# ziyu0425/PDE-Solver

Measured on NVIDIA B200. Metric: GDOF/s, higher is better.
Workload: dtype f64

## Files before the change

### pde_solver_b200/csrc/heat2.cu

```cuda
#include <cuda.h>

#include <cmath>

#include "device.cuh"
#include "tma.cuh"

namespace {

#ifndef H_RR_STAGES
#define H_RR_STAGES 3
#endif
template <bool RR>
struct HS { static constexpr int N = RR ? H_RR_STAGES : 4; };

template <int CW, int YSB>
struct HG {
  static constexpr int TX = CW - 2, YSA = YSB + 1, TY = 2 * YSB, RA = TY + 2;
  static constexpr int BX = TX + 4, BYX = TY + 4, BYB = TY + 2;
  static constexpr int XBOX = BX * BYX, BBOX = BX * BYB;
  static constexpr int XS = (XBOX + 15) / 16 * 16, BS = (BBOX + 15) / 16 * 16;
  static constexpr int STAGE = XS + BS;
  static constexpr int RING = RA * CW;
  static constexpr int NT = 2 * CW;
  static constexpr size_t smem(int nst) { return ((size_t)nst * STAGE + 4 * RING) * sizeof(double) + nst * sizeof(uint64_t); }
};

struct H2Coef {
  double c0, cxp, cxm, cyp, cym, czp, czm, cxyp, cxym, cxzp, cxzm, cyzp, cyzm, cdp, cdm;
};
struct H2Args {
  double* y;
  double a0, a1, k1;
  int do_reduce;
  double* yc;
  int cnn0, cnn1, cnzl, cz0, cPX;
  long long cplane;
};
struct H2Geom {
  int nn0, nn1, nzl, z0, nzg, PX;
  long long plane;
  int ntx, nty, nzc, zc;
};

template <int YS>
__device__ __forceinline__ void h2_contrib(const H2Coef& C, const double (&V)[YS + 2][3], double (&aP)[YS], double (&a0)[YS],
                                           double (&aM)[YS]) {
#pragma unroll
  for (int j = 0; j < YS; ++j) {
    const int r = j + 1;
    double t = fma(C.c0, V[r][1], a0[j]);
    t = fma(C.cxp, V[r][2], t);
    t = fma(C.cxm, V[r][0], t);
    t = fma(C.cyp, V[r + 1][1], t);
    t = fma(C.cym, V[r - 1][1], t);
    t = fma(C.cxyp, V[r + 1][2], t);
    a0[j] = fma(C.cxym, V[r - 1][0], t);
    double p = fma(C.czp, V[r][1], aP[j]);
    p = fma(C.cxzp, V[r][2], p);
    p = fma(C.cyzp, V[r + 1][1], p);
    aP[j] = fma(C.cdp, V[r + 1][2], p);
    double m = C.czm * V[r][1];
    m = fma(C.cxzm, V[r][0], m);
    m = fma(C.cyzm, V[r - 1][1], m);
    aM[j] = fma(C.cdm, V[r - 1][0], m);
  }
}

template <int CW, int YSB, bool RR>
__global__ void __launch_bounds__(2 * CW, CW == 64 ? ((RR && H_RR_STAGES == 3) ? 4 : (YSB >= 4 ? 3 : (YSB == 3 ? 4 : 5))) : 6)
k_heat_post2(const __grid_constant__ CUtensorMap tmx, const __grid_constant__ CUtensorMap tmb,
             const __grid_constant__ H2Coef C, const __grid_constant__ H2Args a, const __grid_constant__ H2Geom ge,
             ReduceBuf red, double* red_out) {
  using G = HG<CW, YSB>;
  constexpr int YSA = G::YSA;
  constexpr int H_STAGES = HS<RR>::N;
  extern __shared__ __align__(128) unsigned char smem_raw[];
  double* const stage0 = reinterpret_cast<double*>(smem_raw);
  double* const ring0 = stage0 + H_STAGES * G::STAGE;
  uint64_t* const bars = reinterpret_cast<uint64_t*>(ring0 + 4 * G::RING);

  const int t = threadIdx.x;
  const int item = blockIdx.x;
  const int itx = item % ge.ntx;
  const int ity = (item / ge.ntx) % ge.nty;
  const int izc = item / (ge.ntx * ge.nty);
  const int x0 = itx * G::TX, y0 = ity * G::TY;
  const int za = izc * ge.zc;
  const int zb = min(za + ge.zc, ge.nzl);
  const int nplanes = zb - za + 4;
  const uint32_t bar0 = smem_u32(bars);
  const uint32_t stg0 = smem_u32(stage0);
  constexpr uint32_t STAGE_BYTES = G::STAGE * 8;

  auto issue = [&](int n) {
    const uint32_t bar = bar0 + 8 * (n % H_STAGES);
    const uint32_t dst = stg0 + (n % H_STAGES) * STAGE_BYTES;
    mbar_expect_tx(bar, (uint32_t)((G::XBOX + (n >= 2 ? G::BBOX : 0)) * 8));
    tma_load_4d(dst, &tmx, x0 - 2, y0 - 2, za - 2 + n + PDE_NG, 0, bar);
    if (n >= 2) tma_load_4d(dst + G::XS * 8, &tmb, x0 - 2, y0 - 1, za - 3 + n + PDE_NG, 0, bar);
  };
  if (t == 0) {
#pragma unroll
    for (int s = 0; s < H_STAGES; ++s) mbar_init(bar0 + 8 * s, 1);
    asm volatile("fence.mbarrier_init.release.cluster;" ::: "memory");
  }
  __syncthreads();
  if (t == 0)
    for (int n = 0; n < 2 && n < nplanes; ++n) issue(n);

  const int c = t % CW;
  const int s = t / CW;
  const int ix = x0 - 1 + c;
  const int cB = min(max(c, 1), CW - 2);
  const bool xfree = ix >= 1 && ix <= ge.nn0 - 2;
  unsigned mAb = 0, mBb = 0, okB = 0;
#pragma unroll
  for (int j = 0; j < YSA; ++j) {
    const int iy = y0 - 1 + s * YSA + j;
    if (xfree && iy >= 1 && iy <= ge.nn1 - 2) mAb |= 1u << j;
  }
#pragma unroll
  for (int j = 0; j < YSB; ++j) {
    const int iy = y0 + s * YSB + j;
    const bool in = c >= 1 && c <= G::TX && ix < ge.nn0 && iy < ge.nn1;
    if (in) okB |= 1u << j;
    if (in && xfree && iy >= 1 && iy <= ge.nn1 - 2) mBb |= 1u << j;
  }
  const int offA = (s * YSA) * G::BX + c;
  const int offbA = G::XS + (s * YSA) * G::BX + c + 1;
  const int offbB = G::XS + (s * YSB + 1) * G::BX + cB + 1;
  const int offxB = (s * YSB + 2) * G::BX + cB + 1;
  const int ringA = (s * YSA) * CW + c;
  const int ringB = (s * YSB) * CW + cB - 1;
  double* yrun = a.y + ((long long)ge.PX * (y0 + s * YSB) + ix) + ge.plane * za;

  double aA[YSA], aB[YSA], aC[YSA];
  double bA_[YSB], bB_[YSB], bC_[YSB];
#pragma unroll
  for (int j = 0; j < YSA; ++j) aA[j] = aB[j] = aC[j] = 0.0;
#pragma unroll
  for (int j = 0; j < YSB; ++j) bA_[j] = bB_[j] = bC_[j] = 0.0;
  double red_by = 0.0;

  auto body = [&](int i, double (&aP)[YSA], double (&a0)[YSA], double (&aM)[YSA], double (&bP)[YSB], double (&b0)[YSB],
                  double (&bM)[YSB]) {
    const int stage = i % H_STAGES;
    const int q = za - 2 + i;
    const int pA = q - 1;
    const int pB = q - 2;
    const bool finA = i >= 2, finB = i >= 4;
    double xB0[YSB], bvB[YSB];
    if (!RR && finB) {
      const double* const sx2 = stage0 + ((i - 2) % H_STAGES) * G::STAGE + offxB;
      const double* const sb1 = stage0 + ((i - 1) % H_STAGES) * G::STAGE + offbB;
#pragma unroll
      for (int j = 0; j < YSB; ++j) { xB0[j] = sx2[j * G::BX]; bvB[j] = sb1[j * G::BX]; }
    }
    mbar_wait(bar0 + 8 * stage, (uint32_t)((i / H_STAGES) & 1));
    const double* const sx = stage0 + stage * G::STAGE;
    {
      double V[YSA + 2][3];
      const double* const sp = sx + offA;
#pragma unroll
      for (int r = 0; r < YSA + 2; ++r)
#pragma unroll
        for (int cc = 0; cc < 3; ++cc)
          V[r][cc] = ((r == 0 && cc == 2) || (r == YSA + 1 && cc == 0)) ? 0.0 : sp[r * G::BX + cc];
      h2_contrib<YSA>(C, V, aP, a0, aM);
    }
    if (finA) {
      const int gz = pA + ge.z0;
      const bool zfree = gz >= 1 && gz <= ge.nzg - 2;
      const unsigned mA = zfree ? mAb : 0u;
      double* const ds = ring0 + ((pA + 4) & 3) * G::RING + ringA;
      const double* const sb = sx + offbA;
#pragma unroll
      for (int j = 0; j < YSA; ++j) ds[j * CW] = ((mA >> j) & 1u) ? a.a0 * (sb[j * G::BX] - aP[j]) : 0.0;
    }
    __syncthreads();
    if (t == 0 && i + 2 < nplanes) issue(i + 2);
    if (!RR && finA) {
      double V[YSB + 2][3];
      const double* const rp = ring0 + ((pA + 4) & 3) * G::RING + ringB;
#pragma unroll
      for (int r = 0; r < YSB + 2; ++r)
#pragma unroll
        for (int cc = 0; cc < 3; ++cc)
          V[r][cc] = ((r == 0 && cc == 2) || (r == YSB + 1 && cc == 0)) ? 0.0 : rp[r * CW + cc];
      h2_contrib<YSB>(C, V, bP, b0, bM);
    }
    if (RR && finB) {
      const int gz = pB + ge.z0;
      const int Z = (gz >> 1) - a.cz0;
      constexpr int NCX = G::TX / 2, NCY = G::TY / 2;
      if (!(gz & 1) && Z >= 0 && Z < a.cnzl && t < NCX * NCY) {
        const int cx = t % NCX, cy = t / NCX;
        const int X = (x0 >> 1) + cx, Y = (y0 >> 1) + cy;
        if (X < a.cnn0 && Y < a.cnn1) {
          const int o = (1 + 2 * cy) * CW + 1 + 2 * cx;
          const double* const r0 = ring0 + ((pB + 4) & 3) * G::RING + o;
          const double* const rm = ring0 + ((pB + 3) & 3) * G::RING + o;
          const double* const rp = ring0 + ((pB + 5) & 3) * G::RING + o;
          const double nb = ((r0[1] + r0[-1]) + (r0[CW] + r0[-CW])) + ((r0[CW + 1] + r0[-CW - 1]) + (rp[0] + rm[0])) +
                            ((rp[1] + rm[-1]) + (rp[CW] + rm[-CW])) + (rp[CW + 1] + rm[-CW - 1]);
          const int cgz = gz >> 1;
          const bool cfree = X >= 1 && X <= a.cnn0 - 2 && Y >= 1 && Y <= a.cnn1 - 2 && cgz >= 1 && cgz <= (ge.nzg >> 1) - 1;
          a.yc[(long long)a.cPX * Y + a.cplane * Z + X] = cfree ? fma(0.5, nb, r0[0]) : 0.0;
        }
      }
    }
    if (!RR && finB) {
      const int gz = pB + ge.z0;
      const bool zfree = gz >= 1 && gz <= ge.nzg - 2;
      const unsigned mB = zfree ? mBb : 0u;
      const double* const dso = ring0 + ((pB + 4) & 3) * G::RING + ringB + CW + 1;
#pragma unroll
      for (int j = 0; j < YSB; ++j) {
        const bool m = (mB >> j) & 1u;
        const double x2 = m ? fma(a.k1, dso[j * CW], fma(-a.a1, bP[j], xB0[j])) : xB0[j];
        if ((okB >> j) & 1u) yrun[j * (long long)ge.PX] = x2;
        red_by = fma(m ? bvB[j] : 0.0, x2, red_by);
      }
      yrun += ge.plane;
    }
  };

  for (int i = 0; i < nplanes; i += 3) {
    body(i, aA, aB, aC, bB_, bC_, bA_);
    if (i + 1 < nplanes) body(i + 1, aB, aC, aA, bC_, bA_, bB_);
    if (i + 2 < nplanes) body(i + 2, aC, aA, aB, bA_, bB_, bC_);
  }
  if (a.do_reduce) {
    double v[1] = {red_by};
    block_reduce_finalize<1>(v, red, red_out);
  }
}

template <int CW, int YSB, bool RR>
int launch_t(pde_ctx* c, const Grid& g, const OpDev& op, const double* x0, const double* b, const H2Args& ha_in) {
  using G = HG<CW, YSB>;
  H2Geom ge;
  ge.nn0 = g.nn[0]; ge.nn1 = g.nn[1]; ge.nzl = g.nzl; ge.z0 = g.z0; ge.nzg = g.nzg; ge.PX = g.PX; ge.plane = g.plane;
  ge.ntx = (g.nn[0] + G::TX - 1) / G::TX;
  ge.nty = (g.nn[1] + G::TY - 1) / G::TY;
  static const int zc_env = env_int("PDE_B200_P2_ZC", 64);
  int zc = zc_env < 4 ? 4 : zc_env;
  while (zc > 8 && (long long)ge.ntx * ge.nty * ((g.nzl + zc - 1) / zc) < 6LL * c->sm_count) zc /= 2;
  ge.nzc = (g.nzl + zc - 1) / zc;
  ge.zc = (g.nzl + ge.nzc - 1) / ge.nzc;
  ge.nzc = (g.nzl + ge.zc - 1) / ge.zc;
  const long long items = (long long)ge.ntx * ge.nty * ge.nzc;
  if (items > RED_MAX_BLOCKS) return 2;
  auto kern = k_heat_post2<CW, YSB, RR>;
  static bool attr_set = false;
  if (!attr_set) {
    CUDA_OK(cudaFuncSetAttribute(kern, cudaFuncAttributeMaxDynamicSharedMemorySize, (int)G::smem(HS<RR>::N)));
    CUDA_OK(cudaFuncSetAttribute(kern, cudaFuncAttributePreferredSharedMemoryCarveout, 100));
    attr_set = true;
  }
  CUtensorMap tmx, tmb;
  PDE_OK(field_tensor_map(x0, g, 1, G::BX, G::BYX, &tmx));
  PDE_OK(field_tensor_map(b, g, 1, G::BX, G::BYB, &tmb));
  H2Coef C;
  const double* h = op.h_int;
  C.c0 = h[0]; C.cxp = h[1]; C.cxm = h[2]; C.cyp = h[3]; C.cym = h[4]; C.czp = h[5]; C.czm = h[6]; C.cxyp = h[7];
  C.cxym = h[8]; C.cxzp = h[9]; C.cxzm = h[10]; C.cyzp = h[11]; C.cyzm = h[12]; C.cdp = h[13]; C.cdm = h[14];
  kern<<<(unsigned)items, G::NT, G::smem(HS<RR>::N), c->stream>>>(tmx, tmb, C, ha_in, ge, c->red, ha_in.do_reduce ? c->scal + ha_in.do_reduce - 1 : nullptr);
  c->launches++;
  CUDA_OK(cudaGetLastError());
  return 0;
}

bool heat2_applicable(const Grid& g, const OpDev& op) {
  static const int off = env_int("PDE_B200_NO_HEAT2", 0);
  if (off) return false;
  if (g.dim != 3 || g.nk != PDE_NOFF || op.ncomp != 1 || !op.uniform_diag) return false;
  return g.nn[0] >= 32 && g.nn[1] >= 8 && g.nzl >= 8;
}

template <bool RR>
int dispatch(pde_ctx* c, const Grid& g, const OpDev& op, const double* x0, const double* b, const H2Args& ha) {
  static const int cw_env = env_int("PDE_B200_P2_CW", 0);
  static const int ysb = env_int("PDE_B200_P2_YSB", 4);
  const int cw = cw_env ? cw_env : (g.nn[0] >= 128 ? 64 : 32);
  if (cw == 64 && ysb == 3) return launch_t<64, 3, RR>(c, g, op, x0, b, ha);
  if (cw == 64) return launch_t<64, 4, RR>(c, g, op, x0, b, ha);
  return launch_t<32, 4, RR>(c, g, op, x0, b, ha);
}

}

bool post2_applicable(const Grid& g, const OpDev& op) {
  if (g.dim != 3 || g.nk != PDE_NOFF || op.ncomp != 1 || !op.uniform_diag) return false;
  if (g.nn[0] < 32 || g.nn[1] < 8 || g.nzl < 8) return false;
  return !env_int("PDE_B200_NO_HEAT2", 0) || !env_int("PDE_B200_NO_POST2", 0);
}

int launch_heat_post2(pde_ctx* c, const Grid& g, const OpDev& op, const double* x0, const double* b, double* y, double c2_0,
                      double c1_1, double c2_1, int dot_slot, bool* handled) {
  *handled = false;
  if (!heat2_applicable(g, op) || !(c2_0 * op.h_dinv_int[0] > 0.0)) return 0;
  H2Args ha{};
  ha.y = y;
  ha.a0 = c2_0 * op.h_dinv_int[0];
  ha.a1 = c2_1 * op.h_dinv_int[0];
  ha.k1 = 1.0 + c1_1 + ha.a1 / ha.a0;
  ha.do_reduce = dot_slot >= 0 ? dot_slot + 1 : 0;
  const int rc = dispatch<false>(c, g, op, x0, b, ha);
  if (rc == 0) *handled = true;
  return rc == 2 ? 0 : rc;
}

int launch_heat_resid_restrict(pde_ctx* c, const Grid& gf, const Grid& gc, const OpDev& op, const double* x, const double* b,
                               double* bcoarse, bool* handled) {
  *handled = false;
  static const int off = env_int("PDE_B200_NO_RR", 0);
  if (off || !heat2_applicable(gf, op)) return 0;
  if (gf.nc[0] != 2 * gc.nc[0] || gf.nc[1] != 2 * gc.nc[1] || gf.nc[2] != 2 * gc.nc[2] || gf.z0 != 2 * gc.z0) return 0;
  H2Args ha{};
  ha.a0 = 1.0;
  ha.yc = bcoarse;
  ha.cnn0 = gc.nn[0]; ha.cnn1 = gc.nn[1]; ha.cnzl = gc.nzl; ha.cz0 = gc.z0; ha.cPX = gc.PX; ha.cplane = gc.plane;
  const int rc = dispatch<true>(c, gf, op, x, b, ha);
  if (rc == 0) *handled = true;
  return rc == 2 ? 0 : rc;
}
```

### pde_solver_b200/csrc/solver.cu

```cuda
#include <cmath>
#include <cstdio>
#include <cstdlib>
#include <cstring>

#include "solver.cuh"

int launch_stencil_generic(pde_ctx* c, const Grid& g, const BcDev& bc, const OpDev& op, const StencilArgs& a);
int launch_stencil_fast(pde_ctx* c, const Grid& g, const BcDev& bc, const OpDev& op, const StencilArgs& a, bool* handled);
int launch_heat_post2(pde_ctx* c, const Grid& g, const OpDev& op, const double* x0, const double* b, double* y, double c2_0,
                      double c1_1, double c2_1, int dot_slot, bool* handled);
bool elast3d_first2_ok(const Grid& g, const BcDev& bc, const OpDev& op);
bool post2_applicable(const Grid& g, const OpDev& op);
int launch_heat_resid_restrict(pde_ctx* c, const Grid& gf, const Grid& gc, const OpDev& op, const double* x, const double* b,
                               double* bcoarse, bool* handled);

int launch_stencil(pde_ctx* c, const Grid& g, const BcDev& bc, const OpDev& op, const StencilArgs& a) {
  if (a.variant == 0) {
    bool handled = false;
    PDE_OK(launch_stencil_fast(c, g, bc, op, a, &handled));
    if (handled) return 0;
  }
  return launch_stencil_generic(c, g, bc, op, a);
}

int Field::alloc(pde_ctx* c, const Grid& g, int ncomp) {
  release();
  const size_t lead = (((size_t)g.PX + 1 + 31) / 32) * 32;
  bytes = ((size_t)g.comp_stride * ncomp + 2 * lead) * sizeof(double);
  CUDA_OK(cudaMalloc(&raw, bytes));
  CUDA_OK(cudaMemsetAsync(raw, 0, bytes, c->stream));
  p = raw + lead + PDE_NG * g.plane;
  return 0;
}
void Field::release() {
  if (raw) cudaFree(raw);
  raw = p = nullptr;
  bytes = 0;
}

int Operator::upload(pde_ctx* c) {
  const int nc = tab.ncomp, nn = nc * nc;
  dev.ncomp = nc;
  dev.gershgorin = tab.gershgorin;
  std::vector<double> dinv((size_t)PDE_NCLASS * nc, 0.0);
  for (int cls = 0; cls < PDE_NCLASS; ++cls)
    for (int i = 0; i < nc; ++i) {
      double dg = tab.coef[((size_t)cls * PDE_NOFF + 0) * nn + i * nc + i];
      dinv[cls * nc + i] = dg > 0 ? 1.0 / dg : 0.0;
    }
  for (int k = 0; k < PDE_NOFF; ++k)
    for (int q = 0; q < nn; ++q) dev.h_int[k * nn + q] = tab.coef[((size_t)13 * PDE_NOFF + k) * nn + q];
  for (int i = 0; i < nc; ++i) dev.h_dinv_int[i] = dinv[13 * nc + i];
  dev.h_load_int = tab.load[13];
  {
    bool u = !bc.side_excl;
    for (int ax = 0; ax < 3; ++ax)
      if (g.nc[ax] > 0 && !(bc.on[2 * ax] && bc.on[2 * ax + 1])) u = false;
    dev.uniform_diag = u ? 1 : 0;
  }
  CUDA_OK(cudaMalloc(&dev.coef, tab.coef.size() * sizeof(double)));
  CUDA_OK(cudaMalloc(&dev.dinv, dinv.size() * sizeof(double)));
  CUDA_OK(cudaMalloc(&dev.load, PDE_NCLASS * sizeof(double)));
  CUDA_OK(cudaMemcpyAsync(dev.coef, tab.coef.data(), tab.coef.size() * sizeof(double), cudaMemcpyHostToDevice, c->stream));
  CUDA_OK(cudaMemcpyAsync(dev.dinv, dinv.data(), dinv.size() * sizeof(double), cudaMemcpyHostToDevice, c->stream));
  CUDA_OK(cudaMemcpyAsync(dev.load, tab.load.data(), PDE_NCLASS * sizeof(double), cudaMemcpyHostToDevice, c->stream));
  CUDA_OK(cudaStreamSynchronize(c->stream));
  return 0;
}
int Operator::setup_scalar(pde_ctx* c, const Grid& g_, const BcDev& bc_, double alpha, double beta) {
  release();
  g = g_;
  bc = bc_;
  PDE_OK(build_scalar_table(g.dim, g.h, g.nc, alpha, beta, &tab));
  return upload(c);
}
int Operator::setup_elasticity(pde_ctx* c, const Grid& g_, const BcDev& bc_, double lam, double mu) {
  release();
  g = g_;
  bc = bc_;
  PDE_OK(build_elasticity_table(g.dim, g.h, g.nc, lam, mu, &tab));
  return upload(c);
}
void Operator::release() {
  if (dev.coef) cudaFree(dev.coef);
  if (dev.dinv) cudaFree(dev.dinv);
  if (dev.load) cudaFree(dev.load);
  dev.coef = dev.dinv = dev.load = nullptr;
}

__global__ void k_publish_scal(const double* __restrict__ src, double* __restrict__ dst_host, int count) {
  if ((int)threadIdx.x < count) dst_host[threadIdx.x] = src[threadIdx.x];
  __threadfence_system();
}
// ... 172 lines not shown
  return 0;
}

int Hierarchy::build(pde_ctx* c, const Operator& fine, int kind, double p0, double p1) {
  release();
  const int dim = fine.g.dim;
  int ax[3], nax;
  internal_axes(dim, ax, &nax);
  int32_t n[3] = {0, 0, 0};
  double Lu[3] = {1, 1, 1};
  for (int q = 0; q < nax; ++q) {
    n[q] = fine.g.nc[ax[q]];
    Lu[q] = fine.g.h[ax[q]] * fine.g.nc[ax[q]];
  }
  const int ncomp = fine.tab.ncomp;
  static const long long rep_nodes = getenv("PDE_B200_REP_NODES") ? atoll(getenv("PDE_B200_REP_NODES")) : 400000;
  bool replicate = false;
  for (int level = 0;; ++level) {
    std::unique_ptr<MGLevel> L(new MGLevel());
    Grid g;
    if (c->world > 1 && level > 0 && !replicate) {
      long long gn = 1;
      for (int q = 0; q < nax; ++q) gn *= (n[q] + 1);
      replicate = gn <= rep_nodes;
    }
    if (replicate) {
      PDE_OK(make_grid(dim, n, Lu, 0, 1, &g));
      if (!lv.back()->replicated) {
        PDE_OK(make_grid(dim, n, Lu, c->rank, c->world, &L->gslab));
        L->gslab.comp_stride = g.comp_stride;
      }
      L->replicated = true;
    } else {
      PDE_OK(make_grid(dim, n, Lu, c->rank, c->world, &g));
    }
    if (kind == PDE_OP_ELASTICITY) PDE_OK(L->op.setup_elasticity(c, g, fine.bc, p0, p1));
    else PDE_OK(L->op.setup_scalar(c, g, fine.bc, p0, p1));
    PDE_OK(L->xa.alloc(c, g, ncomp));
    PDE_OK(L->xb.alloc(c, g, ncomp));
    PDE_OK(L->r.alloc(c, g, ncomp));
    if (level > 0) PDE_OK(L->b.alloc(c, g, ncomp));
    lv.push_back(std::move(L));
    bool can = true;
    if (const char* ml = getenv("PDE_B200_MAX_LEVELS")) can = can && (level + 1 < atoi(ml));
    int32_t nc2[3] = {0, 0, 0};
    static const int env_min = getenv("PDE_B200_MIN_COARSE_CELLS") ? atoi(getenv("PDE_B200_MIN_COARSE_CELLS")) : 0;
    const int min_cells = env_min > 0 ? env_min : (ncomp > 1 ? 2 : 1);
    for (int q = 0; q < nax; ++q) {
      if (n[q] % 2 != 0 || n[q] < 2) can = false;
      nc2[q] = n[q] / 2;
      if (nc2[q] < min_cells) can = false;
    }
    if (c->world > 1 && !replicate && n[nax - 1] % (2 * c->world) != 0) can = false;
    if (can) {
      Grid gc;
      PDE_OK(make_grid(dim, nc2, Lu, 0, 1, &gc));
      long long nodes = (long long)gc.nn[0] * gc.nn[1] * gc.nzl;
      if (nodes <= 200000) {
        long long nfree = count_free_and_index(gc, fine.bc, ncomp, nullptr, nullptr);
        if (nfree <= 0) can = false;
      }
    }
    if (!can) break;
    for (int q = 0; q < nax; ++q) n[q] = nc2[q];
  }
  MGLevel& Lc = *lv.back();
  long long nodes = (long long)Lc.op.g.nn[0] * Lc.op.g.nn[1] * Lc.op.g.nzg;
  if (lv.size() > 1 && nodes * ncomp <= 4 * PDE_DENSE_MAX) {
    Grid gg;
    PDE_OK(make_grid(dim, n, Lu, 0, 1, &gg));
    long long nfree = count_free_and_index(gg, Lc.op.bc, ncomp, nullptr, nullptr);
    if (nfree > 0 && nfree <= PDE_DENSE_MAX) PDE_OK(build_dense_coarse(c, Lc, dim, n, Lu));
  }
  if (ncomp > 1 && !getenv("PDE_B200_NO_LMAX_EST"))
    for (auto& L : lv) PDE_OK(estimate_lmax(c, *L, 12));
  return 0;
}

void Hierarchy::release() {
  if (gexec) cudaGraphExecDestroy(gexec);
  gexec = nullptr;
  gstate = 0;
  gnodes = 0;
  for (auto& L : lv) {
    L->op.release();
    L->b.release(); L->xa.release(); L->xb.release(); L->r.release();
    if (L->Ainv) cudaFree(L->Ainv);
    if (L->idx) cudaFree(L->idx);
    if (L->bglob) cudaFree(L->bglob);
  }
  lv.clear();
}

struct Cheby {
  double theta, delta, sigma, rho, lmax_;
  int kind = 1;
  void init(double lmax, double ratio) {
    static const int env_kind = getenv("PDE_B200_CHEBY_KIND") ? atoi(getenv("PDE_B200_CHEBY_KIND")) : 1;
    kind = env_kind == 4 ? 4 : 1;
    lmax_ = lmax;
    const double lmin = lmax / ratio;
    theta = 0.5 * (lmax + lmin);
    delta = 0.5 * (lmax - lmin);
    sigma = theta / delta;
    rho = 1.0 / sigma;
  }
  void coef(int k, double* c1, double* c2) {
    if (kind == 4) {
      if (k == 0) { *c1 = 0.0; *c2 = 4.0 / (3.0 * lmax_); return; }
      *c1 = (2.0 * k - 1.0) / (2.0 * k + 3.0);
      *c2 = (8.0 * k + 4.0) / ((2.0 * k + 3.0) * lmax_);
      return;
    }
    if (k == 0) { rho = 1.0 / sigma; *c1 = 0.0; *c2 = 1.0 / theta; return; }
    const double rn = 1.0 / (2.0 * sigma - rho);
    *c1 = rn * rho;
    *c2 = 2.0 * rn / delta;
    rho = rn;
  }
};

static int smooth(pde_ctx* c, MGLevel& L, const double* b, double** cur, double** oth, int sweeps, bool zero_guess,
                  double ratio, int dot_slot = -1, bool* dot_done = nullptr, bool halos_valid = false) {
  Cheby ch;
  ch.init(L.op.dev.gershgorin, ratio);
  int k0 = 0;
  int prev_mode = 0;
  double s0 = 0;
  if (dot_done) *dot_done = false;
  const bool e_first2 = !L.op.dev.uniform_diag && dot_slot < 0 && elast3d_first2_ok(L.op.g, L.op.bc, L.op.dev);
  if (zero_guess && sweeps >= 2 && (L.op.dev.uniform_diag || e_first2)) {
    StencilArgs a;
    double c1;
    ch.coef(0, &c1, &s0);
    a.cheby = 2;
    a.s0 = s0;
    ch.coef(1, &a.c1, &a.c2);
    a.x = b; a.y = *cur;
    if (dot_slot >= 0 && sweeps == 2) { a.reduce_slot_xy = dot_slot; if (dot_done) *dot_done = true; }
    if (c->world > 1) PDE_OK(comm_halo_exchange(c, L.op.g, L.op.dev.ncomp, const_cast<double*>(b)));
    PDE_OK(launch_stencil(c, L.op.g, L.op.bc, L.op.dev, a));
    k0 = 2;
    prev_mode = 3;
  } else if (zero_guess) {
    double c1, c2;
    ch.coef(0, &c1, &c2);
    PDE_OK(launch_cheby_first(c, L.op.g, L.op.bc, L.op.dev, b, *cur, c2));
    k0 = 1;
    prev_mode = 2;
  }
  if (!zero_guess && sweeps == 2 && post2_applicable(L.op.g, L.op.dev) && (c->world == 1 || L.op.g.nzl >= PDE_NG)) {
    double c1a, c2a, c1b, c2b;
    ch.coef(0, &c1a, &c2a);
    ch.coef(1, &c1b, &c2b);
    bool handled = false;
    if (c->world > 1 && !halos_valid) {
      PDE_OK(comm_halo_exchange(c, L.op.g, 1, *cur, PDE_NG));
      PDE_OK(comm_halo_exchange(c, L.op.g, 1, const_cast<double*>(b), 1));
    }
    PDE_OK(launch_heat_post2(c, L.op.g, L.op.dev, *cur, b, *oth, c2a, c1b, c2b, dot_slot, &handled));
    if (!handled) PDE_OK(launch_post2(c, L.op.g, L.op.bc, L.op.dev, *cur, b, *oth, c2a, c1b, c2b, dot_slot, &handled));
    if (handled) {
      std::swap(*cur, *oth);
      if (dot_slot >= 0 && dot_done) *dot_done = true;
      return 0;
    }
    ch.init(L.op.dev.gershgorin, ratio);
  }
  for (int k = k0; k < sweeps; ++k) {
    StencilArgs a;
    a.cheby = 1;
    a.x = *cur; a.y = *oth; a.b = b;
    ch.coef(k, &a.c1, &a.c2);
    a.prev_mode = k == 0 ? 0 : prev_mode;
    a.s0 = s0;
    a.xprev = a.prev_mode == 1 ? *oth : nullptr;
    if (dot_slot >= 0 && k == sweeps - 1) { a.reduce_slot_xy = dot_slot; if (dot_done) *dot_done = true; }
    if (c->world > 1) PDE_OK(comm_halo_exchange(c, L.op.g, L.op.dev.ncomp, *cur));
    PDE_OK(launch_stencil(c, L.op.g, L.op.bc, L.op.dev, a));
    std::swap(*cur, *oth);
    prev_mode = 1;
  }
  return 0;
}

int Hierarchy::vcycle(pde_ctx* c, const Operator& fine, const double* b0, double** z_out, int dot_slot,
                      bool* dot_done) {
  if (dot_done) *dot_done = false;
  (void)fine;
  const int nl = (int)lv.size();
  std::vector<double*> cur(nl), oth(nl);
  for (int l = 0; l < nl; ++l) { cur[l] = lv[l]->xa.p; oth[l] = lv[l]->xb.p; }
  std::vector<char> lean(nl, 0);
  for (int l = 0; l + 1 < nl; ++l)
    lean[l] = c->world > 1 && !lv[l]->replicated && nu == 2 && lv[l]->op.dev.uniform_diag && lv[l]->op.dev.ncomp == 1 && lv[l]->op.g.dim == 3 &&
              lv[l]->op.g.nzl >= 8 && lv[l + 1]->op.g.nzl >= PDE_NG && sweep_applicable(lv[l]->op.g, 1) &&
              !getenv("PDE_B200_NO_POST2") && !getenv("PDE_B200_NO_LEAN_HALO");
  auto down = [&](int l) -> int {
    MGLevel& L = *lv[l];
    const double* b = l == 0 ? b0 : L.b.p;
    PDE_OK(smooth(c, L, b, &cur[l], &oth[l], nu, true, ratio));
    if (c->world > 1) PDE_OK(comm_halo_exchange(c, L.op.g, L.op.dev.ncomp, cur[l], lean[l] ? PDE_NG : 1));
    return 0;
  };
  auto restrict_to = [&](int l) -> int {
    MGLevel& L = *lv[l];
    MGLevel& Lc = *lv[l + 1];
    const double* b = l == 0 ? b0 : L.b.p;
    const bool window = Lc.replicated && !L.replicated;
    const Grid& gc = Lc.op.g;
    const int nc = L.op.dev.ncomp;
    if (window) PDE_OK(launch_zero(c, gc, nc, Lc.b.p));
    const Grid& gct = window ? Lc.gslab : gc;
    double* bct = window ? Lc.b.p + gc.plane * Lc.gslab.z0 : Lc.b.p;
    bool fused = false;
    if (c->world == 1 || lean[l]) PDE_OK(launch_heat_resid_restrict(c, L.op.g, gct, L.op.dev, cur[l], b, bct, &fused));
    if (!fused) {
      StencilArgs a;
      a.x = cur[l]; a.b = b; a.y = L.r.p; a.bscale = 1.0; a.ascale = -1.0;
      a.ghost_out = lean[l];
      PDE_OK(launch_stencil(c, L.op.g, L.op.bc, L.op.dev, a));
      if (c->world > 1 && !lean[l]) PDE_OK(comm_halo_exchange(c, L.op.g, nc, L.r.p));
      PDE_OK(launch_restrict(c, L.op.g, gct, Lc.op.bc, nc, L.r.p, bct));
    }
    if (window) PDE_OK(comm_allreduce_buf(c, Lc.b.p, (size_t)(gc.comp_stride * (nc - 1) + gc.plane * gc.nzg)));
    return 0;
  };
  auto coarsest = [&]() -> int {
    MGLevel& L = *lv[nl - 1];
    const double* b = nl == 1 ? b0 : L.b.p;
    if (L.n_dense > 0 && (c->world == 1 || L.replicated)) {
      PDE_OK(launch_dense_solve(c, L.n_dense, L.Ainv, L.idx, b, cur[nl - 1]));
    } else if (L.n_dense > 0) {
      PDE_OK(launch_dense_gather(c, L.n_dense, L.idx, b, L.bglob));
      PDE_OK(comm_allreduce_buf(c, L.bglob, (size_t)L.n_dense));
      PDE_OK(launch_dense_solve_owned(c, L.n_dense, L.Ainv, L.idx, L.bglob, cur[nl - 1]));
    }
    else PDE_OK(smooth(c, L, b, &cur[nl - 1], &oth[nl - 1], nl == 1 ? nu : coarse_sweeps, true, nl == 1 ? ratio : 30.0,
                       nl == 1 ? dot_slot : -1, nl == 1 ? dot_done : nullptr));
    return 0;
  };
  auto prolong_into = [&](int l) -> int {
    MGLevel& L = *lv[l];
    if (c->world > 1) PDE_OK(comm_halo_exchange(c, lv[l + 1]->op.g, L.op.dev.ncomp, cur[l + 1], lean[l] ? PDE_NG : 1));
    PDE_OK(launch_prolong_add(c, L.op.g, lv[l + 1]->op.g, L.op.bc, L.op.dev.ncomp, cur[l + 1], cur[l], lean[l] ? PDE_NG : 0));
    return 0;
  };
  auto post = [&](int l) -> int {
    MGLevel& L = *lv[l];
    const double* b = l == 0 ? b0 : L.b.p;
    PDE_OK(smooth(c, L, b, &cur[l], &oth[l], nu, false, ratio, l == 0 ? dot_slot : -1, l == 0 ? dot_done : nullptr,
                  lean[l] != 0));
    return 0;
  };
  auto sub = [&](int R) -> int {
    for (int l = R; l < nl - 1; ++l) { PDE_OK(down(l)); PDE_OK(restrict_to(l)); }
    PDE_OK(coarsest());
    for (int l = nl - 2; l >= R; --l) { PDE_OK(prolong_into(l)); PDE_OK(post(l)); }
    return 0;
  };
  int R = 1;
  if (c->world > 1) {
    R = nl;
    for (int l = 1; l < nl; ++l)
      if (lv[l]->replicated) { R = l; break; }
  }
  const bool solo = c->world == 1;
  auto graph_part = [&]() -> int {
    if (solo) { PDE_OK(restrict_to(0)); PDE_OK(sub(1)); PDE_OK(prolong_into(0)); return 0; }
    PDE_OK(sub(R));
    return prolong_into(R - 1);
  };
  auto run_graph_part = [&]() -> int {
    if (gstate == 2) {
      CUDA_OK(cudaGraphLaunch(gexec, c->stream));
      c->launches += gnodes;
    } else if (gstate == 1) {
      const long long l0 = c->launches;
      CUDA_OK(cudaStreamBeginCapture(c->stream, cudaStreamCaptureModeThreadLocal));
      const int rc = graph_part();
      cudaGraph_t graph = nullptr;
      const cudaError_t ec = cudaStreamEndCapture(c->stream, &graph);
      if (rc) { if (graph) cudaGraphDestroy(graph); return rc; }
      if (ec != cudaSuccess || !graph) { cudaGetLastError(); gstate = -1; PDE_OK(graph_part()); }
      else {
        gnodes = c->launches - l0;
        const cudaError_t ei = cudaGraphInstantiate(&gexec, graph, 0);
        cudaGraphDestroy(graph);
        if (ei != cudaSuccess) { cudaGetLastError(); gexec = nullptr; gstate = -1; c->launches = l0; PDE_OK(graph_part()); }
        else {
          gstate = 2;
          CUDA_OK(cudaGraphLaunch(gexec, c->stream));
        }
      }
    } else {
      PDE_OK(graph_part());
      if (gstate == 0) gstate = 1;
    }
    return 0;
  };
  if (nl == 1) {
    PDE_OK(coarsest());
    *z_out = cur[0];
    return 0;
  }
  static const int graph_env = getenv("PDE_B200_MG_GRAPH") ? atoi(getenv("PDE_B200_MG_GRAPH")) : 1;
  if (gstate == 0 && !(graph_env && (solo ? nl >= 3 : nl - R >= 2))) gstate = -1;
  PDE_OK(down(0));
  if (solo) {
    PDE_OK(run_graph_part());
  } else {
    PDE_OK(restrict_to(0));
    for (int l = 1; l < R && l < nl - 1; ++l) { PDE_OK(down(l)); PDE_OK(restrict_to(l)); }
    if (R < nl) {
      PDE_OK(run_graph_part());
      for (int l = R - 1; l >= 1; --l) { PDE_OK(post(l)); PDE_OK(prolong_into(l - 1)); }
    } else {
      PDE_OK(coarsest());
      for (int l = nl - 2; l >= 1; --l) { PDE_OK(prolong_into(l)); PDE_OK(post(l)); }
      PDE_OK(prolong_into(0));
    }
  }
  PDE_OK(post(0));
  *z_out = cur[0];
  return 0;
}

int choose_precond(const pde_solver_opts& o, pde_ctx* c, long long ndofs, const Hierarchy& h) {
  if (o.precond == PDE_PRECOND_JACOBI) return PDE_PRECOND_JACOBI;
  if (h.levels() < 2) return PDE_PRECOND_JACOBI;
  if (o.precond == PDE_PRECOND_GMG) return PDE_PRECOND_GMG;
  (void)c;
  return ndofs >= 20000 ? PDE_PRECOND_GMG : PDE_PRECOND_JACOBI;
}

int PcgWork::alloc(pde_ctx* c, const Grid& g, int ncomp) {
  PDE_OK(p.alloc(c, g, ncomp));
  PDE_OK(q.alloc(c, g, ncomp));
  return 0;
}
void PcgWork::release() { p.release(); q.release(); }

int pcg_solve(pde_ctx* c, const Operator& A, Hierarchy* mg, PcgWork& w, double* x, double* r, double bnorm2,
              const pde_solver_opts& o, pde_stats* st) {
  const Grid& g = A.g;
  const int nc = A.dev.ncomp;
  const bool gmg = mg != nullptr;
  const double tol2 = o.rtol * o.rtol * bnorm2;
  st->solves += 1;
  st->levels = gmg ? mg->levels() : 1;
  if (!(bnorm2 > 0.0)) {
    st->final_relres = 0.0;
    return 0;
  }
  double* z = nullptr;
  double rr;
  if (!gmg) {
    CUDA_OK(cudaMemsetAsync(c->scal + S_XY, 0, 2 * sizeof(double), c->stream));
    PDE_OK(launch_cg_update(c, g, A.dev, x, r, w.p.p, w.q.p, S_RHO0, S_XY, S_RHO0, S_RHO0 + 1, 1));
    if (c->world > 1) PDE_OK(comm_allreduce_scal(c, S_RHO0, 2));
    PDE_OK(launch_cg_pupdate(c, g, A.dev, w.p.p, r, S_RHO0, S_RHO0, 1, 1));
  } else {
    bool fused = false;
    PDE_OK(mg->vcycle(c, A, r, &z, S_RHO0, &fused));
    if (!fused) PDE_OK(launch_dot(c, g, nc, r, z, S_RHO0));
    PDE_OK(launch_dot(c, g, nc, r, r, S_RHO0 + 1));
    if (c->world > 1) PDE_OK(comm_allreduce_scal(c, S_RHO0, 2));
    PDE_OK(launch_cg_pupdate(c, g, A.dev, w.p.p, z, S_RHO0, S_RHO0, 1, 0));
  }
  PDE_OK(read_scal(c, S_RHO0 + 1, 1, &rr));
  const bool trace = getenv("PDE_B200_TRACE") != nullptr;
  if (trace) {
    double v[2];
    PDE_OK(read_scal(c, S_RHO0, 2, v));
    fprintf(stderr, "[pcg] n=%lld gmg=%d levels=%d bnorm2=%.6e rho0=%.6e rr0=%.6e\n", (long long)g.total, (int)gmg,
            gmg ? mg->levels() : 1, bnorm2, v[0], v[1]);
  }
  int it = 0;
  bool conv = rr <= tol2;
  const int check = gmg ? 1 : (o.check_every > 0 ? o.check_every : 10);
  while (!conv && it < o.max_iters) {
    const int sr = 2 * (it & 1), sn = 2 * (1 - (it & 1));
    StencilArgs a;
    a.x = w.p.p; a.y = w.q.p; a.reduce_slot_xy = S_XY;
    a.skip_yy = 1;
    if (c->world > 1) PDE_OK(comm_halo_exchange(c, g, nc, w.p.p));
    PDE_OK(launch_stencil(c, g, A.bc, A.dev, a));
    if (c->world > 1) PDE_OK(comm_allreduce_scal(c, S_XY, 1));
    PDE_OK(launch_cg_update(c, g, A.dev, gmg ? nullptr : x, r, w.p.p, w.q.p, sr, S_XY, sn, sn + 1, !gmg));
    if (c->world > 1 && !gmg) PDE_OK(comm_allreduce_scal(c, sn, 2));
    if (gmg) {
      bool fused = false;
      PDE_OK(mg->vcycle(c, A, r, &z, sn, &fused));
      if (!fused) PDE_OK(launch_dot(c, g, nc, r, z, sn));
      if (c->world > 1) PDE_OK(comm_allreduce_scal(c, sn, 2));
    }
    PDE_OK(launch_cg_pupdate(c, g, A.dev, w.p.p, gmg ? z : r, sr, sn, 0, !gmg, gmg ? x : nullptr, S_XY));
    ++it;
    if (trace && (it <= 30 || it % 50 == 0)) {
      double v[2], pap;
      PDE_OK(read_scal(c, sn, 2, v));
      PDE_OK(read_scal(c, S_XY, 1, &pap));
      fprintf(stderr, "[pcg] it=%d pAp=%.6e rho=%.6e rr=%.6e\n", it, pap, v[0], v[1]);
    }
    if (it % check == 0 || it >= o.max_iters) {
      PDE_OK(read_scal(c, sn + 1, 1, &rr));
// ... 10 lines not shown
```

### pde_solver_b200/csrc/solver.cuh

```cuda
#pragma once
#include <memory>

#include "device.cuh"

struct Field {
  double* raw = nullptr;
  double* p = nullptr;
  size_t bytes = 0;
  int alloc(pde_ctx* c, const Grid& g, int ncomp);
  void release();
};

struct Operator {
  Grid g{};
  BcDev bc{};
  OpDev dev{};
  OpTable tab;
  int setup_scalar(pde_ctx* c, const Grid& g, const BcDev& bc, double alpha, double beta);
  int setup_elasticity(pde_ctx* c, const Grid& g, const BcDev& bc, double lam, double mu);
  int upload(pde_ctx* c);
  void release();
};

struct MGLevel {
  Operator op;
  Field b, xa, xb, r;
  bool replicated = false;
  Grid gslab{};
  int n_dense = 0;
  double* Ainv = nullptr;
  long long* idx = nullptr;
  double* bglob = nullptr;
};

struct Hierarchy {
  std::vector<std::unique_ptr<MGLevel>> lv;
  int nu = 2;
  double ratio = 8.0;
  int coarse_sweeps = 8;
  int build(pde_ctx* c, const Operator& fine, int kind, double p0, double p1);
  int vcycle(pde_ctx* c, const Operator& fine, const double* b0, double** z_out, int dot_slot = -1,
             bool* dot_done = nullptr);
  int levels() const { return (int)lv.size(); }
  void release();
  cudaGraphExec_t gexec = nullptr;
  int gstate = 0;
  long long gnodes = 0;
};

struct PcgWork {
  Field p, q;
  int alloc(pde_ctx* c, const Grid& g, int ncomp);
  void release();
};

int pcg_solve(pde_ctx* c, const Operator& A, Hierarchy* mg, PcgWork& w, double* x, double* r, double bnorm2,
              const pde_solver_opts& o, pde_stats* st);

int project_trig_ic(pde_ctx* c, const Grid& g, const BcDev& bc, int dim, const int32_t n_user[3], const double L_user[3],
                    const double* lo_user, double amp, double kw, int use_sin, const pde_solver_opts& o, double* u,
                    double* rhs);
int read_scal(pde_ctx* c, int slot, int count, double* out);
int choose_precond(const pde_solver_opts& o, pde_ctx* c, long long ndofs, const Hierarchy& h);
```

Measured before the change: 2.571.

## Fold multigrid prolongation into the fused heat post-smoothing kernel

The separate prolong_add launch before post-smoothing is replaced by loading the coarse correction via TMA into a small shared-memory ring. Each fine plane gets the trilinear correction added in shared memory before the stencil runs. This saves a full fine-grid read-modify-write pass and a kernel launch per level. In exchange it adds a block-wide sync and async-proxy fence per plane, more shared memory (which may lower occupancy), and reworks the V-cycle and CUDA-graph control flow.

```diff
diff --git a/pde_solver_b200/csrc/heat2.cu b/pde_solver_b200/csrc/heat2.cu
--- a/pde_solver_b200/csrc/heat2.cu
+++ b/pde_solver_b200/csrc/heat2.cu
@@ -22,7 +22,12 @@
   static constexpr int STAGE = XS + BS;
   static constexpr int RING = RA * CW;
   static constexpr int NT = 2 * CW;
-  static constexpr size_t smem(int nst) { return ((size_t)nst * STAGE + 4 * RING) * sizeof(double) + nst * sizeof(uint64_t); }
+  static constexpr int NPF = (XBOX + NT - 1) / NT;
+  static constexpr int CBX = CW / 2 + 4, CBY = TY / 2 + 3;
+  static constexpr int CBOX = CBX * CBY, CS = (CBOX + 15) / 16 * 16;
+  static constexpr size_t smem(int nst, bool pf) {
+    return ((size_t)nst * STAGE + 4 * RING + (pf ? 3 * CS : 0)) * sizeof(double) + nst * sizeof(uint64_t);
+  }
 };
 
 struct H2Coef {
@@ -66,18 +71,21 @@
   }
 }
 
-template <int CW, int YSB, bool RR>
+template <int CW, int YSB, bool RR, bool PF>
 __global__ void __launch_bounds__(2 * CW, CW == 64 ? ((RR && H_RR_STAGES == 3) ? 4 : (YSB >= 4 ? 3 : (YSB == 3 ? 4 : 5))) : 6)
 k_heat_post2(const __grid_constant__ CUtensorMap tmx, const __grid_constant__ CUtensorMap tmb,
-             const __grid_constant__ H2Coef C, const __grid_constant__ H2Args a, const __grid_constant__ H2Geom ge,
+             const __grid_constant__ CUtensorMap tmc, const __grid_constant__ H2Coef C, const __grid_constant__ H2Args a,
+             const __grid_constant__ H2Geom ge,
              ReduceBuf red, double* red_out) {
+  static_assert(!(RR && PF), "the prolongation fold belongs to the post sweeps");
   using G = HG<CW, YSB>;
   constexpr int YSA = G::YSA;
   constexpr int H_STAGES = HS<RR>::N;
   extern __shared__ __align__(128) unsigned char smem_raw[];
   double* const stage0 = reinterpret_cast<double*>(smem_raw);
   double* const ring0 = stage0 + H_STAGES * G::STAGE;
-  uint64_t* const bars = reinterpret_cast<uint64_t*>(ring0 + 4 * G::RING);
+  double* const cring = ring0 + 4 * G::RING;
+  uint64_t* const bars = reinterpret_cast<uint64_t*>(cring + (PF ? 3 * G::CS : 0));
 
   const int t = threadIdx.x;
   const int item = blockIdx.x;
@@ -91,13 +99,19 @@
   const uint32_t bar0 = smem_u32(bars);
   const uint32_t stg0 = smem_u32(stage0);
   constexpr uint32_t STAGE_BYTES = G::STAGE * 8;
+  const int cx0 = ((x0 - 2) >> 1) & ~1;
 
   auto issue = [&](int n) {
     const uint32_t bar = bar0 + 8 * (n % H_STAGES);
     const uint32_t dst = stg0 + (n % H_STAGES) * STAGE_BYTES;
-    mbar_expect_tx(bar, (uint32_t)((G::XBOX + (n >= 2 ? G::BBOX : 0)) * 8));
+    const int gzn = za - 2 + n + ge.z0;
+    const int clo = !PF ? 0 : (n == 0 ? gzn >> 1 : (gzn + 1) >> 1);
+    const int chi = !PF ? -1 : (n == 0 || (gzn & 1) ? (gzn + 1) >> 1 : clo - 1);
+    mbar_expect_tx(bar, (uint32_t)((G::XBOX + (n >= 2 ? G::BBOX : 0) + (chi - clo + 1) * G::CBOX) * 8));
     tma_load_4d(dst, &tmx, x0 - 2, y0 - 2, za - 2 + n + PDE_NG, 0, bar);
     if (n >= 2) tma_load_4d(dst + G::XS * 8, &tmb, x0 - 2, y0 - 1, za - 3 + n + PDE_NG, 0, bar);
+    for (int z = clo; z <= chi; ++z)
+      tma_load_4d(smem_u32(cring + ((z + 3) % 3) * G::CS), &tmc, cx0, (y0 >> 1) - 1, z - a.cz0 + PDE_NG, 0, bar);
   };
   if (t == 0) {
 #pragma unroll
@@ -133,6 +147,15 @@
   const int ringA = (s * YSA) * CW + c;
   const int ringB = (s * YSB) * CW + cB - 1;
   double* yrun = a.y + ((long long)ge.PX * (y0 + s * YSB) + ix) + ge.plane * za;
+  unsigned pfm = 0;
+  if (PF) {
+#pragma unroll
+    for (int k = 0; k < G::NPF; ++k) {
+      const int e = t + k * G::NT;
+      const int fx = x0 - 2 + e % G::BX, fy = y0 - 2 + e / G::BX;
+      if (e < G::XBOX && fx >= 1 && fx <= ge.nn0 - 2 && fy >= 1 && fy <= ge.nn1 - 2) pfm |= 1u << k;
+    }
+  }
 
   double aA[YSA], aB[YSA], aC[YSA];
   double bA_[YSB], bB_[YSB], bC_[YSB];
@@ -157,6 +180,24 @@
       for (int j = 0; j < YSB; ++j) { xB0[j] = sx2[j * G::BX]; bvB[j] = sb1[j * G::BX]; }
     }
     mbar_wait(bar0 + 8 * stage, (uint32_t)((i / H_STAGES) & 1));
+    const int pgz = q + ge.z0;
+    if (PF && pgz >= 1 && pgz <= ge.nzg - 2) {
+      const double* const cf = cring + (((pgz >> 1) + 3) % 3) * G::CS;
+      const double* const cu = cring + ((((pgz + 1) >> 1) + 3) % 3) * G::CS;
+      const int d = ((x0 - 2) >> 1) - cx0;
+      double* const bxp = stage0 + stage * G::STAGE;
+      unsigned tv;
+      asm volatile("mov.u32 %0, %%tid.x;" : "=r"(tv));
+#pragma unroll
+      for (int k = 0; k < G::NPF; ++k) {
+        const int e = (int)tv + k * G::NT;
+        const int by = e / G::BX, bx = e - by * G::BX;
+        const int o = (by >> 1) * G::CBX + d + (bx >> 1);
+        if ((pfm >> k) & 1u) bxp[e] += 0.5 * (cf[o] + cu[o + (by & 1) * G::CBX + (bx & 1)]);
+      }
+      asm volatile("fence.proxy.async.shared::cta;" ::: "memory");
+      __syncthreads();
+    }
     const double* const sx = stage0 + stage * G::STAGE;
     {
       double V[YSA + 2][3];
@@ -236,8 +277,9 @@
   }
 }
 
-template <int CW, int YSB, bool RR>
-int launch_t(pde_ctx* c, const Grid& g, const OpDev& op, const double* x0, const double* b, const H2Args& ha_in) {
+template <int CW, int YSB, bool RR, bool PF>
+int launch_t(pde_ctx* c, const Grid& g, const OpDev& op, const double* x0, const double* b, const H2Args& ha_in,
+             const Grid* gc, const double* ec) {
   using G = HG<CW, YSB>;
   H2Geom ge;
   ge.nn0 = g.nn[0]; ge.nn1 = g.nn[1]; ge.nzl = g.nzl; ge.z0 = g.z0; ge.nzg = g.nzg; ge.PX = g.PX; ge.plane = g.plane;
@@ -251,21 +293,23 @@
   ge.nzc = (g.nzl + ge.zc - 1) / ge.zc;
   const long long items = (long long)ge.ntx * ge.nty * ge.nzc;
   if (items > RED_MAX_BLOCKS) return 2;
-  auto kern = k_heat_post2<CW, YSB, RR>;
+  auto kern = k_heat_post2<CW, YSB, RR, PF>;
   static bool attr_set = false;
   if (!attr_set) {
-    CUDA_OK(cudaFuncSetAttribute(kern, cudaFuncAttributeMaxDynamicSharedMemorySize, (int)G::smem(HS<RR>::N)));
+    CUDA_OK(cudaFuncSetAttribute(kern, cudaFuncAttributeMaxDynamicSharedMemorySize, (int)G::smem(HS<RR>::N, PF)));
     CUDA_OK(cudaFuncSetAttribute(kern, cudaFuncAttributePreferredSharedMemoryCarveout, 100));
     attr_set = true;
   }
-  CUtensorMap tmx, tmb;
+  CUtensorMap tmx, tmb, tmc;
   PDE_OK(field_tensor_map(x0, g, 1, G::BX, G::BYX, &tmx));
   PDE_OK(field_tensor_map(b, g, 1, G::BX, G::BYB, &tmb));
+  if (PF) PDE_OK(field_tensor_map(ec, *gc, 1, G::CBX, G::CBY, &tmc));
+  else tmc = tmx;
   H2Coef C;
   const double* h = op.h_int;
   C.c0 = h[0]; C.cxp = h[1]; C.cxm = h[2]; C.cyp = h[3]; C.cym = h[4]; C.czp = h[5]; C.czm = h[6]; C.cxyp = h[7];
   C.cxym = h[8]; C.cxzp = h[9]; C.cxzm = h[10]; C.cyzp = h[11]; C.cyzm = h[12]; C.cdp = h[13]; C.cdm = h[14];
-  kern<<<(unsigned)items, G::NT, G::smem(HS<RR>::N), c->stream>>>(tmx, tmb, C, ha_in, ge, c->red, ha_in.do_reduce ? c->scal + ha_in.do_reduce - 1 : nullptr);
+  kern<<<(unsigned)items, G::NT, G::smem(HS<RR>::N, PF), c->stream>>>(tmx, tmb, tmc, C, ha_in, ge, c->red, ha_in.do_reduce ? c->scal + ha_in.do_reduce - 1 : nullptr);
   c->launches++;
   CUDA_OK(cudaGetLastError());
   return 0;
@@ -278,14 +322,15 @@
   return g.nn[0] >= 32 && g.nn[1] >= 8 && g.nzl >= 8;
 }
 
-template <bool RR>
-int dispatch(pde_ctx* c, const Grid& g, const OpDev& op, const double* x0, const double* b, const H2Args& ha) {
+template <bool RR, bool PF>
+int dispatch(pde_ctx* c, const Grid& g, const OpDev& op, const double* x0, const double* b, const H2Args& ha,
+             const Grid* gc = nullptr, const double* ec = nullptr) {
   static const int cw_env = env_int("PDE_B200_P2_CW", 0);
   static const int ysb = env_int("PDE_B200_P2_YSB", 4);
   const int cw = cw_env ? cw_env : (g.nn[0] >= 128 ? 64 : 32);
-  if (cw == 64 && ysb == 3) return launch_t<64, 3, RR>(c, g, op, x0, b, ha);
-  if (cw == 64) return launch_t<64, 4, RR>(c, g, op, x0, b, ha);
-  return launch_t<32, 4, RR>(c, g, op, x0, b, ha);
+  if (cw == 64 && ysb == 3) return launch_t<64, 3, RR, PF>(c, g, op, x0, b, ha, gc, ec);
+  if (cw == 64) return launch_t<64, 4, RR, PF>(c, g, op, x0, b, ha, gc, ec);
+  return launch_t<32, 4, RR, PF>(c, g, op, x0, b, ha, gc, ec);
 }
 
 }
@@ -297,16 +342,18 @@
 }
 
 int launch_heat_post2(pde_ctx* c, const Grid& g, const OpDev& op, const double* x0, const double* b, double* y, double c2_0,
-                      double c1_1, double c2_1, int dot_slot, bool* handled) {
+                      double c1_1, double c2_1, int dot_slot, const Grid* gc, const double* ec, bool* handled) {
   *handled = false;
   if (!heat2_applicable(g, op) || !(c2_0 * op.h_dinv_int[0] > 0.0)) return 0;
+  if (ec && (g.nc[0] != 2 * gc->nc[0] || g.nc[1] != 2 * gc->nc[1] || g.nc[2] != 2 * gc->nc[2])) return 0;
   H2Args ha{};
   ha.y = y;
   ha.a0 = c2_0 * op.h_dinv_int[0];
   ha.a1 = c2_1 * op.h_dinv_int[0];
   ha.k1 = 1.0 + c1_1 + ha.a1 / ha.a0;
   ha.do_reduce = dot_slot >= 0 ? dot_slot + 1 : 0;
-  const int rc = dispatch<false>(c, g, op, x0, b, ha);
+  if (ec) ha.cz0 = gc->z0;
+  const int rc = ec ? dispatch<false, true>(c, g, op, x0, b, ha, gc, ec) : dispatch<false, false>(c, g, op, x0, b, ha);
   if (rc == 0) *handled = true;
   return rc == 2 ? 0 : rc;
 }
@@ -321,7 +368,7 @@
   ha.a0 = 1.0;
   ha.yc = bcoarse;
   ha.cnn0 = gc.nn[0]; ha.cnn1 = gc.nn[1]; ha.cnzl = gc.nzl; ha.cz0 = gc.z0; ha.cPX = gc.PX; ha.cplane = gc.plane;
-  const int rc = dispatch<true>(c, gf, op, x, b, ha);
+  const int rc = dispatch<true, false>(c, gf, op, x, b, ha);
   if (rc == 0) *handled = true;
   return rc == 2 ? 0 : rc;
 }
diff --git a/pde_solver_b200/csrc/solver.cu b/pde_solver_b200/csrc/solver.cu
--- a/pde_solver_b200/csrc/solver.cu
+++ b/pde_solver_b200/csrc/solver.cu
@@ -8,7 +8,7 @@
 int launch_stencil_generic(pde_ctx* c, const Grid& g, const BcDev& bc, const OpDev& op, const StencilArgs& a);
 int launch_stencil_fast(pde_ctx* c, const Grid& g, const BcDev& bc, const OpDev& op, const StencilArgs& a, bool* handled);
 int launch_heat_post2(pde_ctx* c, const Grid& g, const OpDev& op, const double* x0, const double* b, double* y, double c2_0,
-                      double c1_1, double c2_1, int dot_slot, bool* handled);
+                      double c1_1, double c2_1, int dot_slot, const Grid* gc, const double* ec, bool* handled);
 bool elast3d_first2_ok(const Grid& g, const BcDev& bc, const OpDev& op);
 bool post2_applicable(const Grid& g, const OpDev& op);
 int launch_heat_resid_restrict(pde_ctx* c, const Grid& gf, const Grid& gc, const OpDev& op, const double* x, const double* b,
@@ -347,6 +347,7 @@
   gexec = nullptr;
   gstate = 0;
   gnodes = 0;
+  gres = nullptr;
   for (auto& L : lv) {
     L->op.release();
     L->b.release(); L->xa.release(); L->xb.release(); L->r.release();
@@ -385,8 +386,18 @@
   }
 };
 
+struct Fold {
+  const Grid* gc;
+  const double* e;
+  int ghost;
+};
+
 static int smooth(pde_ctx* c, MGLevel& L, const double* b, double** cur, double** oth, int sweeps, bool zero_guess,
-                  double ratio, int dot_slot = -1, bool* dot_done = nullptr, bool halos_valid = false) {
+                  double ratio, int dot_slot = -1, bool* dot_done = nullptr, bool halos_valid = false,
+                  const Fold* pf = nullptr) {
+  auto prolong = [&]() -> int {
+    return launch_prolong_add(c, L.op.g, *pf->gc, L.op.bc, L.op.dev.ncomp, pf->e, *cur, pf->ghost);
+  };
   Cheby ch;
   ch.init(L.op.dev.gershgorin, ratio);
   int k0 = 0;
@@ -414,7 +425,9 @@
     k0 = 1;
     prev_mode = 2;
   }
-  if (!zero_guess && sweeps == 2 && post2_applicable(L.op.g, L.op.dev) && (c->world == 1 || L.op.g.nzl >= PDE_NG)) {
+  const bool post2 = !zero_guess && sweeps == 2 && post2_applicable(L.op.g, L.op.dev) && (c->world == 1 || L.op.g.nzl >= PDE_NG);
+  if (pf && !post2) PDE_OK(prolong());
+  if (post2) {
     double c1a, c2a, c1b, c2b;
     ch.coef(0, &c1a, &c2a);
     ch.coef(1, &c1b, &c2b);
@@ -423,7 +436,9 @@
       PDE_OK(comm_halo_exchange(c, L.op.g, 1, *cur, PDE_NG));
       PDE_OK(comm_halo_exchange(c, L.op.g, 1, const_cast<double*>(b), 1));
     }
-    PDE_OK(launch_heat_post2(c, L.op.g, L.op.dev, *cur, b, *oth, c2a, c1b, c2b, dot_slot, &handled));
+    PDE_OK(launch_heat_post2(c, L.op.g, L.op.dev, *cur, b, *oth, c2a, c1b, c2b, dot_slot, pf ? pf->gc : nullptr,
+                             pf ? pf->e : nullptr, &handled));
+    if (!handled && pf) PDE_OK(prolong());
     if (!handled) PDE_OK(launch_post2(c, L.op.g, L.op.bc, L.op.dev, *cur, b, *oth, c2a, c1b, c2b, dot_slot, &handled));
     if (handled) {
       std::swap(*cur, *oth);
@@ -505,23 +520,36 @@
                        nl == 1 ? dot_slot : -1, nl == 1 ? dot_done : nullptr));
     return 0;
   };
+  static const bool no_fold = getenv("PDE_B200_NO_FOLD") != nullptr;
+  std::vector<char> fold(nl, 0);
+  for (int l = 0; l + 1 < nl; ++l) fold[l] = !no_fold && (c->world == 1 || lv[l]->replicated);
+  auto coarse_halo = [&](int l) -> int {
+    if (c->world > 1) PDE_OK(comm_halo_exchange(c, lv[l + 1]->op.g, lv[l]->op.dev.ncomp, cur[l + 1], lean[l] ? PDE_NG : 1));
+    return 0;
+  };
   auto prolong_into = [&](int l) -> int {
     MGLevel& L = *lv[l];
-    if (c->world > 1) PDE_OK(comm_halo_exchange(c, lv[l + 1]->op.g, L.op.dev.ncomp, cur[l + 1], lean[l] ? PDE_NG : 1));
+    PDE_OK(coarse_halo(l));
     PDE_OK(launch_prolong_add(c, L.op.g, lv[l + 1]->op.g, L.op.bc, L.op.dev.ncomp, cur[l + 1], cur[l], lean[l] ? PDE_NG : 0));
     return 0;
   };
-  auto post = [&](int l) -> int {
+  auto post = [&](int l, const Fold* pf) -> int {
     MGLevel& L = *lv[l];
     const double* b = l == 0 ? b0 : L.b.p;
     PDE_OK(smooth(c, L, b, &cur[l], &oth[l], nu, false, ratio, l == 0 ? dot_slot : -1, l == 0 ? dot_done : nullptr,
-                  lean[l] != 0));
-    return 0;
+                  lean[l] != 0, pf));
+    return 0;
+  };
+  auto up = [&](int l) -> int {
+    if (!fold[l]) { PDE_OK(prolong_into(l)); return post(l, nullptr); }
+    PDE_OK(coarse_halo(l));
+    const Fold f{&lv[l + 1]->op.g, cur[l + 1], lean[l] ? PDE_NG : 0};
+    return post(l, &f);
   };
   auto sub = [&](int R) -> int {
     for (int l = R; l < nl - 1; ++l) { PDE_OK(down(l)); PDE_OK(restrict_to(l)); }
     PDE_OK(coarsest());
-    for (int l = nl - 2; l >= R; --l) { PDE_OK(prolong_into(l)); PDE_OK(post(l)); }
+    for (int l = nl - 2; l >= R; --l) PDE_OK(up(l));
     return 0;
   };
   int R = 1;
@@ -531,15 +559,18 @@
       if (lv[l]->replicated) { R = l; break; }
   }
   const bool solo = c->world == 1;
+  const int Rb = solo ? 1 : R;
   auto graph_part = [&]() -> int {
-    if (solo) { PDE_OK(restrict_to(0)); PDE_OK(sub(1)); PDE_OK(prolong_into(0)); return 0; }
-    PDE_OK(sub(R));
-    return prolong_into(R - 1);
+    if (solo) { PDE_OK(restrict_to(0)); PDE_OK(sub(1)); }
+    else PDE_OK(sub(R));
+    return fold[Rb - 1] ? 0 : prolong_into(Rb - 1);
   };
   auto run_graph_part = [&]() -> int {
     if (gstate == 2) {
       CUDA_OK(cudaGraphLaunch(gexec, c->stream));
       c->launches += gnodes;
+      cur[Rb] = gres;
+      return 0;
     } else if (gstate == 1) {
       const long long l0 = c->launches;
       CUDA_OK(cudaStreamBeginCapture(c->stream, cudaStreamCaptureModeThreadLocal));
@@ -562,6 +593,7 @@
       PDE_OK(graph_part());
       if (gstate == 0) gstate = 1;
     }
+    gres = cur[Rb];
     return 0;
   };
   if (nl == 1) {
@@ -572,21 +604,17 @@
   static const int graph_env = getenv("PDE_B200_MG_GRAPH") ? atoi(getenv("PDE_B200_MG_GRAPH")) : 1;
   if (gstate == 0 && !(graph_env && (solo ? nl >= 3 : nl - R >= 2))) gstate = -1;
   PDE_OK(down(0));
-  if (solo) {
-    PDE_OK(run_graph_part());
-  } else {
+  if (!solo) {
     PDE_OK(restrict_to(0));
     for (int l = 1; l < R && l < nl - 1; ++l) { PDE_OK(down(l)); PDE_OK(restrict_to(l)); }
-    if (R < nl) {
-      PDE_OK(run_graph_part());
-      for (int l = R - 1; l >= 1; --l) { PDE_OK(post(l)); PDE_OK(prolong_into(l - 1)); }
-    } else {
-      PDE_OK(coarsest());
-      for (int l = nl - 2; l >= 1; --l) { PDE_OK(prolong_into(l)); PDE_OK(post(l)); }
-      PDE_OK(prolong_into(0));
-    }
-  }
-  PDE_OK(post(0));
+  }
+  if (solo || R < nl) {
+    PDE_OK(run_graph_part());
+    for (int l = Rb - 1; l >= 0; --l) PDE_OK(l == Rb - 1 && !fold[l] ? post(l, nullptr) : up(l));
+  } else {
+    PDE_OK(coarsest());
+    for (int l = nl - 2; l >= 0; --l) PDE_OK(up(l));
+  }
   *z_out = cur[0];
   return 0;
 }
diff --git a/pde_solver_b200/csrc/solver.cuh b/pde_solver_b200/csrc/solver.cuh
--- a/pde_solver_b200/csrc/solver.cuh
+++ b/pde_solver_b200/csrc/solver.cuh
@@ -46,6 +46,7 @@
   cudaGraphExec_t gexec = nullptr;
   int gstate = 0;
   long long gnodes = 0;
+  double* gres = nullptr;
 };
 
 struct PcgWork {
```

New measurement: 2.691, median of 6. 1.05x the previous value.
